# pySTEPS/pysteps

Hardware: AMD Instinct MI355X
Metric: Mpixels*leadsteps/s (LK+semilag) at 4096x4096 fp32 (higher is better)
Workload: dtype f32

## Files before the change

include/pysteps_hip.h:

```cpp
#ifndef PYSTEPS_HIP_H
#define PYSTEPS_HIP_H

#include <stddef.h>
#include <stdint.h>

#ifdef __cplusplus
extern "C" {
#endif

#define PSH_OK 0
#define PSH_EINVAL (-1)
#define PSH_EHIP (-2)
#define PSH_ENOTINIT (-3)
#define PSH_ENOMEM (-4)
#define PSH_ECOMM (-5)
#define PSH_EUNSUPPORTED (-6)
#define PSH_EINPUT (-7)

int psh_init(int device_id);
int psh_shutdown(void);
const char *psh_last_error(void);
const char *psh_version(void);
int psh_device_info(int *device_id, int *cu_count, size_t *hbm_total, size_t *hbm_free,
                    char *name, int name_len);
// ... 254 lines not shown
typedef struct psh_lk_params {
  int size_opening;
  int buffer_mask;
  int max_corners;
  int block_size;
  double quality_level, min_distance;
  int win_w, win_h;
  int max_level;
  int max_count;
  double epsilon;
  double min_eig_threshold;
  double nr_std_outlier;
  int k_outlier;
  double decl_scale;
  int idw_k;
  double idw_power, idw_dist_offset;
  int frames_f64;
} psh_lk_params;
int psh_dense_lk_dev(const float *frames_dev, int nframes, int m, int n, const psh_lk_params *params,
                     float *field_dev, double *xy_host, double *uv_host, int capacity,
                     int *count_out);
int psh_dense_lk_uv_dev(const float *frames_dev, int nframes, int m, int n, const psh_lk_params *params,
                        float *field_dev, float *field_uv_dev, double *xy_host, double *uv_host, int capacity,
                        int *count_out);

int psh_outliers_local_host(const double *xy, const double *values, int n, int k, double thr,
                            unsigned char *flags);

int psh_decluster_host(const double *xy, const double *values, int n, double scale,
                       int min_samples, double *out_xy, double *out_values, int *out_count);
int psh_vectors_finish_host(const double *xy, const double *values, const unsigned char *outlier_flags,
                            int count, double decl_scale, int m, int n, float *out_xy, float *out_values,
                            int *out_count, int *out_mode, float *out_const, float *out_reach);

int psh_fft_rfft2_dev(const double *in_dev, int m, int n, void *out_dev);
int psh_fft_irfft2_dev(const void *in_dev, int m, int n, double *out_dev);
int psh_fft_irfft2_min_dev(const void *in_dev, int m, int n, double *out_dev, unsigned long long *min_key_dev);
int psh_fft_c2c2_dev(const void *in_dev, int m, int n, int inverse, void *out_dev);

int psh_cascade_decompose_dev(const double *field_dev, const double *weights_dev, int nlevels, int m, int n,
                              int normalize, int subtract_mean, double *levels_dev, double *means_host,
                              double *stds_host, double *field_mean_host);
int psh_cascade_decompose_stats_dev(const double *field_dev, const double *weights_dev, int nlevels, int m, int n,
                                    double *levels_dev, double *stats_dev);
int psh_cascade_decompose_levels_dev(const double *field_dev, const double *weights_dev, int nlevels, int m, int n,
                                     double *levels_dev);
int psh_cascade_recompose_dev(const double *levels_dev, int nlevels, int m, int n, const double *means_host,
                              const double *stds_host, double field_mean, double *out_dev);
int psh_noise_filter_dev(const double *white_dev, const double *filter_dev, int m, int n, double *out_dev);
int psh_ar_iterate_dev(const double *x_dev, int nt, size_t plane, const double *phi_host, int p,
                       const double *eps_dev, double *out_dev);

int psh_probmatch_dev(const double *initial_dev, const double *target_dev, size_t count, double *out_dev);
int psh_probmatch_async_dev(const double *initial_dev, const double *target_dev, size_t count, double *out_dev,
                            int *status_dev);
int psh_probmatch_status(int status);
int psh_order_statistic_dev(const double *field_dev, size_t count, size_t index, double *value_host);
int psh_probmatch_plan_create(const double *target_dev, size_t count, void **plan_out);
int psh_probmatch_plan_destroy(void *plan);
int psh_probmatch_planned_dev(const void *plan, const double *initial_dev, size_t count, double *out_dev, int *status_dev);
int psh_steps_mask_probmatch_dev(const void *plan, double *field_dev, size_t count, const double *grey_mask_dev,
                                 const unsigned char *keep_mask_dev, const unsigned long long *min_key_dev,
                                 double *out_dev, int *status_dev);

int psh_dilated_mask_dev(const unsigned char *mask_dev, int m, int n, const unsigned char *kr_host, int kh, int kw,
                         int r, double *out_dev);
// ... 89 lines not shown
```

pysteps_amd/_lib.py:

```python

import ctypes
import os
import threading

from ctypes import POINTER, c_char_p, c_double, c_float, c_int, c_size_t, c_void_p

_PKG = os.path.dirname(os.path.abspath(__file__))
LIB_PATH = os.environ.get("PYSTEPS_HIP_LIB") or os.path.join(_PKG, "lib", "libpysteps_hip.so")

PSH_OK = 0
PSH_EINVAL = -1
PSH_EHIP = -2
PSH_ENOTINIT = -3
PSH_ENOMEM = -4
PSH_ECOMM = -5
PSH_EUNSUPPORTED = -6
PSH_EINPUT = -7


class LkParams(ctypes.Structure):

    _fields_ = [
        ("size_opening", c_int), ("buffer_mask", c_int), ("max_corners", c_int), ("block_size", c_int),
        ("quality_level", c_double), ("min_distance", c_double),
# ... 191 lines not shown
    "psh_lk_track_pyr_dev": (c_int, [c_void_p, c_void_p, c_int, c_int, c_double, c_double, c_void_p, c_void_p]),
    "psh_db_transform_dev": (c_int, [c_void_p, c_void_p, c_size_t, c_double, c_double, c_int]),
    "psh_field_transform_dev": (c_int, [c_void_p, c_void_p, c_int, c_size_t, c_int, c_double, c_double, c_double, c_double]),
    "psh_nqt_count_le_dev": (c_int, [c_void_p, c_int, c_size_t, c_void_p, c_void_p, POINTER(c_size_t), POINTER(c_double),
                                     POINTER(c_double), POINTER(c_float)]),
    "psh_nqt_forward_dev": (c_int, [c_void_p, c_int, c_void_p, c_size_t, c_size_t, c_double, c_double, c_void_p, c_int,
                                    POINTER(c_double)]),
    "psh_nqt_table_dev": (c_int, [c_size_t, c_double, c_void_p]),
    "psh_nqt_inverse_dev": (c_int, [c_void_p, c_int, c_size_t, c_void_p, c_void_p, c_int, c_size_t, c_void_p, c_int,
                                    POINTER(c_double), POINTER(c_double)]),
    "psh_nonfinite_count_f64_dev": (c_int, [c_void_p, c_size_t, POINTER(c_double)]),
    "psh_field_stats_dev": (c_int, [c_void_p, c_size_t, POINTER(c_double), POINTER(c_double), POINTER(c_double), POINTER(c_double)]),
    "psh_dense_lk_dev": (c_int, [c_void_p, c_int, c_int, c_int, POINTER(LkParams), c_void_p, c_void_p, c_void_p, c_int, POINTER(c_int)]),
    "psh_dense_lk_uv_dev": (c_int, [c_void_p, c_int, c_int, c_int, POINTER(LkParams), c_void_p, c_void_p, c_void_p, c_void_p, c_int,
                                    POINTER(c_int)]),
    "psh_semilag_dev": (c_int, [c_void_p, c_void_p, c_int, c_int, c_void_p, c_int, c_int, c_int, c_float, c_void_p, c_int, c_void_p]),
    "psh_semilag_uv_dev": (c_int, [c_void_p, c_void_p, c_void_p, c_int, c_int, c_void_p, c_int, c_int, c_int, c_float, c_void_p, c_int,
                                   c_void_p]),
    "psh_semilag_window_shape": (c_int, [c_int, c_int]),
    "psh_semilag_kernel": (c_int, [c_int, c_int, c_int, c_int, c_int, c_int]),
    "psh_semilag_rows_dev": (c_int, [c_void_p, c_void_p, c_int, c_int, c_void_p, c_int, c_int, c_int, c_float, c_void_p, c_int, c_int, c_int, c_void_p]),
    "psh_semilag_host": (c_int, [c_void_p, c_void_p, c_int, c_int, c_void_p, c_int, c_int, c_int, c_float, c_void_p, c_void_p, c_void_p, c_int, POINTER(c_int)]),
}

DIMENSION_SIGNATURES = {
    "psh_aggregate_axis_dev": (c_int, [c_void_p, c_int, c_size_t, c_size_t, c_size_t, c_int, c_int, c_int, c_void_p]),
    "psh_aggregate_space_dev": (c_int, [c_void_p, c_int, c_size_t, c_int, c_int, c_int, c_int, c_int, c_int, c_void_p]),
    "psh_accumulate_step_dev": (c_int, [c_void_p, c_int, c_void_p, c_int, c_void_p, c_size_t, c_int, c_int, c_int, c_int]),
    "psh_window_copy_dev": (c_int, [c_void_p, c_int, c_size_t, c_int, c_int, c_int, c_int, c_void_p, c_int, c_int, c_int, c_int, c_int,
                                    c_int, c_int, c_double]),
    "psh_field_min_dev": (c_int, [c_void_p, c_int, c_size_t, POINTER(c_double)]),
}

_lock = threading.RLock()
_lib = None
_initialised = False


def load():
    global _lib
    with _lock:
        if _lib is not None:
            return _lib
        if not os.path.exists(LIB_PATH):
            raise HipLibraryError(
                "libpysteps_hip.so not found at %s - build it with "
                "`python -m pysteps_amd.build` (hipcc, gfx950). pysteps_amd has no CPU fallback."
                % LIB_PATH
            )
        try:
            lib = ctypes.CDLL(LIB_PATH)
        except OSError as exc:
            raise HipLibraryError("cannot load %s: %s" % (LIB_PATH, exc)) from exc
        for name, (restype, argtypes) in list(SIGNATURES.items()) + list(DIMENSION_SIGNATURES.items()):
            try:
                fn = getattr(lib, name)
            except AttributeError as exc:
                raise HipLibraryError("%s does not export %s" % (LIB_PATH, name)) from exc
            fn.restype = restype
            fn.argtypes = argtypes
        _lib = lib
        return lib


def last_error():
    msg = load().psh_last_error()
    return msg.decode("utf-8", "replace") if msg else ""


def check(rc, what=""):
    if rc == PSH_OK:
        return
    msg = "%s%s" % (what + ": " if what else "", last_error())
    if rc in (PSH_EINVAL, PSH_EINPUT):
        raise ValueError(msg)
    if rc == PSH_EUNSUPPORTED:
        raise NotImplementedError(msg)
    if rc == PSH_ENOMEM:
        raise MemoryError(msg)
    raise HipLibraryError(msg)


def default_device():
    for key in ("PYSTEPS_HIP_DEVICE", "LOCAL_RANK"):
        val = os.environ.get(key)
        if val not in (None, ""):
            return int(val)
# ... 13 lines not shown
```

pysteps_amd/csrc/common.h:

```cpp
#pragma once

#include <hip/hip_runtime.h>

#include <cmath>
#include <cstdarg>
#include <cstddef>
#include <cstdint>
#include <cstdio>
#include <mutex>

#include "../../include/pysteps_hip.h"
#include "entry.h"
#include "scratch.h"

#ifdef PSH_DEBUG
#include <cassert>
#define PSH_DASSERT(cond) assert(cond)
#else
#define PSH_DASSERT(cond) ((void)0)
#endif

namespace psh {

constexpr int kNumXcd = 8;
// ... 94 lines not shown
                            int npad = 0, int pad_edge = 0, float cval = 0.f, int order = 3);

struct IdwDyn {
  int L;
  int mode;
  float cu, cv;
  float reach;
  int pad[3];
};

bool fft_shape_supported(int m, int n);
int fft_irfft2_weighted(const void *spec_dev, const double *weights_dev, int m, int n, double *out_dev,
                        void *scratch_dev, unsigned long long *min_key_dev = nullptr);

int moments(const double *x_dev, int planes, size_t plane, double2 *stats_dev, hipStream_t stream);

struct IdwArgs {
  const float *xy;
  const float *uv;
  float *out;
  float *out_uv = nullptr;
  int L, k, m, n;
  float x0, dx, y0, dy;
  float inv_res, power, offset, dmax;
  void *scratch = nullptr;
  const IdwDyn *dyn = nullptr;
};
hipError_t launch_idw(const IdwArgs &a, hipStream_t stream);
int idw_resident(const float *xy_dev, const float *values_dev, int capacity, const IdwDyn *dyn_dev, int m, int n,
                 int k, double power, double dist_offset, float *out_dev, float *out_uv_dev = nullptr);
size_t idw_scratch_bytes(int m, int n);
void set_idw_variant(int v);

hipError_t launch_outliers_pooled(const double *xy_dev, const double *uv_dev, const int *count_dev,
                                  int capacity, int k, double thr, unsigned char *flags_dev,
                                  hipStream_t stream);
int lk_track_pool(void *pyramid_handle, const float *points_host, const float *points_dev, const int *npts_dev,
                  int npts, int max_count, double epsilon, double min_eig_threshold, double *pool_xy_dev,
                  double *pool_uv_dev, int *pool_count_dev, int pool_capacity);

int lk_corners_resident(const unsigned char *feature_u8_dev, const float *clean_dev, float *stats_dev, int m, int n,
                        int block_size, int buffer_mask, double quality_level, double min_distance, int max_corners,
                        float *points_dev, int *npoints_dev, int (*before_walk)(void *) = nullptr,
                        void *before_walk_arg = nullptr, int *walk_stats_host = nullptr,
                        unsigned *slots_cleared = nullptr);

size_t lk_prepare_ws_bytes(int m, int n, bool f64);
int lk_prepare_on(hipStream_t stream, void *ws, const void *frame_dev, bool f64, int m, int n, int size_opening,
                  int buffer_mask, float *clean_dev, unsigned char *track_u8_dev, unsigned char *feature_u8_dev,
                  float *stats_dev, unsigned *slots_cleared = nullptr, unsigned long long *keepbits = nullptr);
size_t lk_keepbits_bytes(int m, int n);
size_t lk_slot_bytes();
int lk_pyramids_on_side(hipStream_t side, void *block, size_t block_bytes, const unsigned char *prev_u8_dev,
                        const unsigned char *next_u8_dev, int m, int n, int win_w, int win_h, int max_level,
                        void **handle_out);
size_t lk_pyramids_bytes(int m, int n, int win_w, int win_h, int max_level);

int corner_order_max_corners();
bool corner_order_supported(int m, int n, double min_distance, int max_corners);
size_t corner_order_ws_bytes();
hipError_t launch_corner_order(const unsigned long long *raw_dev, const int *raw_count_dev, int cap,
                               const float *eig_max_dev, float quality, int n, double min_distance,
                               int max_corners, void *ws_dev, float *points_dev, int *npoints_dev,
                               hipStream_t stream, int (*before_walk)(void *), void *before_walk_arg,
                               bool ws_is_cleared, const unsigned *eig_slots_dev = nullptr, int count_bias = 0,
                               float *eig_max_out_dev = nullptr);
size_t corner_order_clear_bytes();
size_t corner_order_walk_stats_offset();
hipError_t launch_vectors_finish(const double *pool_xy_dev, const double *pool_uv_dev,
                                 const unsigned char *flags_dev, const int *pool_count_dev, int capacity,
                                 double decl_scale, int m, int n, float *xy_out_dev, float *uv_out_dev,
                                 IdwDyn *dyn_dev, hipStream_t stream);

}
```

pysteps_amd/csrc/dense_lk.hip:

```cpp
#include <algorithm>
#include <chrono>
#include <cmath>
#include <cstdio>
#include <cstdlib>
#include <cstring>
#include <vector>

#include "common.h"

namespace {

__global__ __launch_bounds__(256) void zero_dwords(unsigned *__restrict__ p, size_t n) {
  for (size_t i = threadIdx.x; i < n; i += 256) p[i] = 0u;
}

}

extern "C" int psh_dense_lk_uv_dev(const float *frames_dev, int nframes, int m, int n, const psh_lk_params *prm,
                                   float *field_dev, float *field_uv_dev, double *xy_host, double *uv_host, int capacity,
                                   int *count_out);

extern "C" int psh_dense_lk_dev(const float *frames_dev, int nframes, int m, int n,
                                const psh_lk_params *prm, float *field_dev, double *xy_host,
                                double *uv_host, int capacity, int *count_out) {
// ... 83 lines not shown
    const int rc1 = psh::lk_corners_resident(feat[t].as<unsigned char>(), nan_pattern(t),
                                             stats[t].as<float>(), m, n, prm->block_size, prm->buffer_mask,
                                             prm->quality_level, prm->min_distance, prm->max_corners, d_pts, d_npts,
                                             nullptr, nullptr, trace ? walk_stats : nullptr, frame_slots(t));
    if (int rc = prepare(t + 1, side, ws_side.as<void>())) {
      (void)psh::side_end();
      return rc;
    }
    struct Fork {
      void *pyr;
      int rc;
    } fork{nullptr, PSH_OK};
    fork.rc = psh::lk_pyramids_on_side(side, pyr_block.release(), pyr_bytes, trk[t].as<unsigned char>(), trk[t + 1].as<unsigned char>(),
                                       m, n, prm->win_w, prm->win_h, prm->max_level, &fork.pyr);
    const int rcj = psh::side_end();
    void *pyr = fork.pyr;
    if (trace)
      std::fprintf(stderr,
                   "dense_lk corner walk: %d chunk(s), %d candidates, %d evaluation(s) of the first wave; us: load %d sort %d "
                   "coordinates %d block tests %d survivors %d (cells %d - evaluations %d append %d) total %d\n",
                   walk_stats[0], walk_stats[1], walk_stats[2], walk_stats[3], walk_stats[4], walk_stats[5],
                   walk_stats[6], walk_stats[7], walk_stats[9], walk_stats[11], walk_stats[12], walk_stats[8]);
    if (rc1 || rcj || fork.rc || !pyr) {
      if (pyr) (void)psh_lk_pyramids_free(pyr);
      return fork.rc ? fork.rc : rc1 ? rc1 : rcj ? rcj : psh::fail(PSH_EHIP, "dense_lk: pyramids were not built");
    }
    const int rc2 = psh::lk_track_pool(pyr, nullptr, d_pts, d_npts, prm->max_corners, prm->max_count, prm->epsilon,
                                       prm->min_eig_threshold, d_pxy, d_puv, d_pcnt, capacity_dev);
    const int rc3 = psh_lk_pyramids_free(pyr);
    if (rc2) return rc2;
    if (rc3) return rc3;
  }
  mark("pairs queued");
  PSH_HIP(psh::launch_outliers_pooled(d_pxy, d_puv, d_pcnt, capacity_dev, prm->k_outlier, prm->nr_std_outlier,
                                      d_pfl, c.stream));
  if (field_dev) {
    psh::Scratch samples;
    const size_t sbytes = cap * 2 * sizeof(float);
    if (int rc = samples.alloc(2 * sbytes + 256)) return rc;
    float *d_xy = samples.as<float>(), *d_uv = d_xy + cap * 2;
    psh::IdwDyn *d_dyn = samples.at<psh::IdwDyn>(2 * sbytes);
    PSH_HIP(psh::launch_vectors_finish(d_pxy, d_puv, d_pfl, d_pcnt, capacity_dev, prm->decl_scale, m, n, d_xy, d_uv,
                                       d_dyn, c.stream));
    if (int rc = psh::idw_resident(d_xy, d_uv, capacity_dev, d_dyn, m, n, prm->idw_k, prm->idw_power,
                                   prm->idw_dist_offset, field_dev, field_uv_dev))
      return rc;
    mark("dense field queued");
    if (count_out) {
      static void *pinned_cnt = nullptr;
      if (int rc = psh::persistent_pinned(&pinned_cnt, 64)) return rc;
      PSH_HIP(hipMemcpyAsync(pinned_cnt, &d_dyn->L, sizeof(int), hipMemcpyDeviceToHost, c.stream));
      PSH_HIP(hipStreamSynchronize(c.stream));
      *count_out = *static_cast<const int *>(pinned_cnt);
    }
    return PSH_OK;
  }

  static void *pinned = nullptr;
  constexpr size_t kPinBytes = 2 * 8192 * 16 + 256 + 8192;
  if (int rc = psh::persistent_pinned(&pinned, kPinBytes)) return rc;
  char *pin = static_cast<char *>(pinned);
  PSH_HIP(hipMemcpyAsync(pin, pbase, off_fl + cap, hipMemcpyDeviceToHost, c.stream));
  PSH_HIP(hipStreamSynchronize(c.stream));
  mark("pooled vectors on the host");
  const int pooled = std::min(*reinterpret_cast<const int *>(pin + off_cnt), capacity_dev);
  const double *hxy = reinterpret_cast<const double *>(pin);
  const double *huv = reinterpret_cast<const double *>(pin + off_uv);
  const unsigned char *hfl = reinterpret_cast<const unsigned char *>(pin + off_fl);
  int count = 0;
  for (int i = 0; i < pooled; ++i) {
    if (pooled >= 2 && hfl[i]) continue;
    if (count >= capacity)
      return psh::fail(PSH_EINVAL, "dense_lk: the vectors exceed the output capacity %d", capacity);
    xy_host[2 * count] = hxy[2 * i];
    xy_host[2 * count + 1] = hxy[2 * i + 1];
    uv_host[2 * count] = huv[2 * i];
// ... 7 lines not shown
```

pysteps_amd/csrc/lk_sparse.hip:

```cpp
#include <cstddef>

#include "common.h"

namespace psh {
namespace {

using CornerKey = unsigned long long;

constexpr int kOrdThreads = 1024;
constexpr int kOrdWaves = kOrdThreads / 64;
constexpr int kOrdBins = 1024;
constexpr int kChunkCap = 4096;
constexpr int kMaxCornersDev = 2048;
constexpr int kHashSlots = 8192;

template <bool DESC>
__device__ __forceinline__ void bitonic_sort_lds(unsigned long long *keys, int p2) {
  for (int k = 2; k <= p2; k <<= 1) {
    for (int j = k >> 1; j > 0; j >>= 1) {
      for (int t = threadIdx.x; t < (p2 >> 1); t += blockDim.x) {
        const int i = ((t & ~(j - 1)) << 1) | (t & (j - 1)), o = i | j;
        const unsigned long long a = keys[i], b = keys[o];
        const bool first_half = (i & k) == 0;
        if ((first_half == DESC) ? a < b : a > b) {
          keys[i] = b;
          keys[o] = a;
        }
      }
      const int next_j = j > 1 ? (j >> 1) : k;
      if (j > 64 || next_j > 64 || (k == p2 && j == 1)) {
        __syncthreads();
      } else {
        __builtin_amdgcn_fence(__ATOMIC_RELEASE, "wavefront");
        __builtin_amdgcn_wave_barrier();
        __builtin_amdgcn_fence(__ATOMIC_ACQUIRE, "wavefront");
// ... 601 lines not shown
      lap(tk_batch);
    }
    remaining -= cnt;
    if (T <= key_lo) break;
    upper = T;
    __syncthreads();
  }
  if (tid == 0) {
    *npoints = nacc;
    if (hdr) {
      hdr->walk[0] = st_chunks;
      hdr->walk[1] = st_walked;
      hdr->walk[2] = st_batches;
      const long long tk[6] = {tk_load, tk_sort, tk_xy, tk_test, tk_batch, wall_clock64() - tk_start};
      for (int q = 0; q < 6; ++q) hdr->phase_us[q] = static_cast<int>(tk[q] / 100);
      for (int q = 0; q < 4; ++q) hdr->sub_us[q] = static_cast<int>(tk_sub[q] / 100);
    }
  }
}

constexpr int kFinMax = 8192;

__device__ __forceinline__ double wave_min_f64(double v) {
#pragma unroll
  for (int d = 32; d >= 1; d >>= 1) v = fmin(v, __shfl_xor(v, d));
  return v;
}
__device__ __forceinline__ double wave_max_f64(double v) {
#pragma unroll
  for (int d = 32; d >= 1; d >>= 1) v = fmax(v, __shfl_xor(v, d));
  return v;
}

__global__ __launch_bounds__(kOrdThreads) void vectors_finish(const double2 *__restrict__ pool_xy,
                                                              const double2 *__restrict__ pool_uv,
                                                              const unsigned char *__restrict__ flags,
                                                              const int *__restrict__ pool_count, int capacity,
                                                              double scale, int m, int n,
                                                              float2 *__restrict__ out_xy,
                                                              float2 *__restrict__ out_uv,
                                                              IdwDyn *__restrict__ dyn) {
  __shared__ unsigned long long s_keys[kFinMax];
  __shared__ unsigned short s_seg[kFinMax];
  __shared__ int s_scan[kOrdWaves];
  __shared__ double s_stat[6][kOrdWaves];
  __shared__ double s_first[2];
  const int tid = threadIdx.x, lane = tid & 63, wave = tid >> 6;
  const int pooled = min(max(*pool_count, 0), min(capacity, kFinMax));
  const bool decl = scale > 1.0;
  constexpr unsigned long long kDropped = ~0ull;
  const int p2 = next_pow2(pooled);
  for (int i = tid; i < p2; i += kOrdThreads) {
    unsigned long long key = kDropped;
    if (i < pooled && !(pooled >= 2 && flags[i])) {
      unsigned cellkey = 0u;
      if (decl) {
        const double2 p = pool_xy[i];
        const double fx = floor(p.x / scale), fy = floor(p.y / scale);
        const unsigned cx = static_cast<unsigned>(fmin(fmax(fx, 0.0), 65535.0));
        const unsigned cy = static_cast<unsigned>(fmin(fmax(fy, 0.0), 65535.0));
        cellkey = (cx << 16) | cy;
      }
      key = decl ? (static_cast<unsigned long long>(cellkey) << 32) | static_cast<unsigned>(i)
                 : static_cast<unsigned long long>(i) << 32 | static_cast<unsigned>(i);
    }
    s_keys[i] = key;
  }
  __syncthreads();
  bitonic_sort_lds<false>(s_keys, p2);
  const int per = max(p2 / kOrdThreads, 1);
  const int t0 = tid * per;
  int heads = 0, kept_here = 0;
  for (int q = 0; q < per; ++q) {
    const int t = t0 + q;
    if (t >= p2) break;
    const unsigned long long k = s_keys[t];
    if (k == kDropped) continue;
    ++kept_here;
    if (t == 0 || (s_keys[t - 1] >> 32) != (k >> 32)) ++heads;
  }
  int incl = heads;
#pragma unroll
  for (int d = 1; d < 64; d <<= 1) {
    const int up = __shfl_up(incl, d);
    if (lane >= d) incl += up;
  }
  if (lane == 63) s_scan[wave] = incl;
  __syncthreads();
  int before = incl - heads, cells = 0;
  for (int w = 0; w < kOrdWaves; ++w) {
    if (w < wave) before += s_scan[w];
    cells += s_scan[w];
  }
  {
    int slot = before - 1;
    for (int q = 0; q < per; ++q) {
      const int t = t0 + q;
      if (t >= p2) break;
      const unsigned long long k = s_keys[t];
      if (k == kDropped) continue;
      if (t == 0 || (s_keys[t - 1] >> 32) != (k >> 32)) ++slot;
      s_seg[t] = static_cast<unsigned short>(slot);
    }
  }
  (void)kept_here;
  __syncthreads();
  double vmin = INFINITY, vmax = -INFINITY;
  double xmin = 0.0, xmax = static_cast<double>(n) - 1.0, ymin = 0.0, ymax = static_cast<double>(m) - 1.0;
  for (int t = tid; t < p2; t += kOrdThreads) {
    const unsigned long long k = s_keys[t];
    if (k == kDropped) continue;
    const unsigned cellkey = static_cast<unsigned>(k >> 32);
    int s = t, e = t + 1;
    while (s > 0 && static_cast<unsigned>(s_keys[s - 1] >> 32) == cellkey) --s;
    while (e < p2 && static_cast<unsigned>(s_keys[e] >> 32) == cellkey) ++e;
    const int members = e - s;
    const int me = static_cast<int>(k & 0xffffffffull);
    const double2 mxy = pool_xy[me], muv = pool_uv[me];
    const double mine[4] = {mxy.x, mxy.y, muv.x, muv.y};
    int rank[4] = {0, 0, 0, 0};
    double succ[4] = {INFINITY, INFINITY, INFINITY, INFINITY};
    for (int q = s; q < e; ++q) {
      if (q == t) continue;
      const int o = static_cast<int>(s_keys[q] & 0xffffffffull);
      const double2 oxy = pool_xy[o], ouv = pool_uv[o];
      const double other[4] = {oxy.x, oxy.y, ouv.x, ouv.y};
#pragma unroll
      for (int c = 0; c < 4; ++c) {
        const bool below = other[c] < mine[c] || (other[c] == mine[c] && q < t);
        rank[c] += below ? 1 : 0;
        if (!below) succ[c] = fmin(succ[c], other[c]);
      }
    }
    const int lower = (members - 1) / 2;
    const bool even = (members & 1) == 0;
    const int slot = s_seg[t];
    double med[4];
    bool have[4];
#pragma unroll
    for (int c = 0; c < 4; ++c) {
      have[c] = rank[c] == lower;
      med[c] = 0.5 * (mine[c] + (even ? succ[c] : mine[c]));
    }
    if (have[0]) {
      reinterpret_cast<float *>(out_xy)[2 * slot] = static_cast<float>(med[0]);
      xmin = fmin(xmin, med[0]);
      xmax = fmax(xmax, med[0]);
    }
    if (have[1]) {
      reinterpret_cast<float *>(out_xy)[2 * slot + 1] = static_cast<float>(med[1]);
      ymin = fmin(ymin, med[1]);
      ymax = fmax(ymax, med[1]);
    }
    if (have[2]) {
      reinterpret_cast<float *>(out_uv)[2 * slot] = static_cast<float>(med[2]);
      vmin = fmin(vmin, med[2]);
      vmax = fmax(vmax, med[2]);
      if (slot == 0) s_first[0] = med[2];
// ... 60 lines not shown
hipError_t launch_corner_order(const unsigned long long *raw_dev, const int *raw_count_dev, int cap,
                               const float *eig_max_dev, float quality, int n, double min_distance,
                               int max_corners, void *ws_dev, float *points_dev, int *npoints_dev,
                               hipStream_t stream, int (*before_walk)(void *), void *before_walk_arg,
                               bool ws_is_cleared, const unsigned *eig_slots_dev, int count_bias, float *eig_max_out_dev) {
  const int cell = static_cast<int>(std::lrint(min_distance)) > 1 ? static_cast<int>(std::lrint(min_distance)) : 1;
  const double md2 = std::ceil(min_distance * min_distance);
  const unsigned md2_ceil = md2 >= 2147483647.0 ? 2147483647u : static_cast<unsigned>(md2);
  char *ws = static_cast<char *>(ws_dev);
  int *hist = reinterpret_cast<int *>(ws);
  OrderHeader *hdr = reinterpret_cast<OrderHeader *>(ws + kOrdOffHdr);
  CornerKey *head = reinterpret_cast<CornerKey *>(ws + kOrdOffHead);
  if (!ws_is_cleared) {
    const hipError_t e = hipMemsetAsync(ws, 0, kOrdOffHead, stream);
    if (e != hipSuccess) return e;
  }
  const int groups = std::max(1, std::min(128, (cap + 4 * kPreThreads - 1) / (4 * kPreThreads)));
  hipLaunchKernelGGL(corner_hist, dim3(groups), dim3(kPreThreads), 0, stream, raw_dev, raw_count_dev, cap, eig_max_dev,
                     quality, hist, eig_slots_dev, count_bias);
  int ccap = 1024;
  while (ccap < 2 * max_corners && ccap < kChunkCap) ccap <<= 1;
  hipLaunchKernelGGL(corner_gather, dim3(groups), dim3(kPreThreads), 0, stream, raw_dev, raw_count_dev, cap, eig_max_dev,
                     quality, hist, head, hdr, ccap, eig_slots_dev, count_bias);
  if (before_walk != nullptr && before_walk(before_walk_arg) != 0) return hipErrorUnknown;
  hipLaunchKernelGGL(corner_order, dim3(1), dim3(kOrdThreads), 0, stream, raw_dev, raw_count_dev, cap, eig_max_dev,
                     quality, head, hdr, n, cell, md2_ceil, min_distance >= 1.0 ? 1 : 0, max_corners, ccap,
                     reinterpret_cast<float2 *>(points_dev), npoints_dev, eig_slots_dev, count_bias, eig_max_out_dev);
  return hipGetLastError();
}

hipError_t launch_vectors_finish(const double *pool_xy_dev, const double *pool_uv_dev,
                                 const unsigned char *flags_dev, const int *pool_count_dev, int capacity,
                                 double decl_scale, int m, int n, float *xy_out_dev, float *uv_out_dev,
                                 IdwDyn *dyn_dev, hipStream_t stream) {
  hipLaunchKernelGGL(vectors_finish, dim3(1), dim3(kOrdThreads), 0, stream,
                     reinterpret_cast<const double2 *>(pool_xy_dev), reinterpret_cast<const double2 *>(pool_uv_dev),
                     flags_dev, pool_count_dev, capacity, decl_scale, m, n, reinterpret_cast<float2 *>(xy_out_dev),
                     reinterpret_cast<float2 *>(uv_out_dev), dyn_dev);
  return hipGetLastError();
}

}

extern "C" int psh_lk_order_host(const unsigned long long *keys_host, int count, float response_max,
                                 double quality_level, int m, int n, double min_distance, int max_corners,
                                 float *points_host, int *count_host) {
  PSH_ENTER(c);
  if (!points_host || !count_host || (count > 0 && !keys_host)) return psh::fail(PSH_EINVAL, "lk_order: NULL pointer");
  if (count < 0 || m <= 0 || n <= 0 || max_corners <= 0) return psh::fail(PSH_EINVAL, "lk_order: invalid argument");
  if (!psh::corner_order_supported(m, n, min_distance, max_corners))
    return psh::fail(PSH_EUNSUPPORTED, "lk_order: more than %d corners, 65535 rows / columns or min_distance >= 16383",
                     psh::kMaxCornersDev);
  const size_t key_bytes = (static_cast<size_t>(count) * sizeof(unsigned long long) + 255) & ~static_cast<size_t>(255);
  const size_t pts_bytes = static_cast<size_t>(max_corners) * 2 * sizeof(float);
  psh::Scratch blk;
  const size_t ws_bytes = (psh::corner_order_ws_bytes() + 255) & ~static_cast<size_t>(255);
  if (int rc = blk.alloc(key_bytes + 256 + pts_bytes + 256 + ws_bytes)) return rc;
  char *base = blk.as<char>();
  unsigned long long *d_keys = reinterpret_cast<unsigned long long *>(base);
  int *d_hdr = reinterpret_cast<int *>(base + key_bytes);
  float *d_pts = reinterpret_cast<float *>(base + key_bytes + 256);
  void *d_ws = base + ((key_bytes + 256 + pts_bytes + 255) & ~static_cast<size_t>(255));
  struct {
    int count, accepted;
    float top;
  } hdr = {count, 0, response_max};
  if (count > 0) PSH_HIP(hipMemcpyAsync(d_keys, keys_host, static_cast<size_t>(count) * 8, hipMemcpyHostToDevice, c.stream));
  PSH_HIP(hipMemcpyAsync(d_hdr, &hdr, sizeof(hdr), hipMemcpyHostToDevice, c.stream));
  PSH_HIP(hipStreamSynchronize(c.stream));
  PSH_HIP(psh::launch_corner_order(d_keys, d_hdr, count, reinterpret_cast<const float *>(d_hdr + 2),
                                   static_cast<float>(quality_level), n, min_distance, max_corners, d_ws, d_pts,
// ... 24 lines not shown
  const size_t vec = cap * 16, off_uv = vec, off_fl = 2 * vec, off_cnt = (off_fl + cap + 255) & ~static_cast<size_t>(255);
  const size_t off_oxy = off_cnt + 256, off_ouv = off_oxy + cap * 8, off_dyn = off_ouv + cap * 8;
  psh::Scratch blk;
  if (int rc = blk.alloc(off_dyn + sizeof(psh::IdwDyn))) return rc;
  char *base = blk.as<char>();
  if (count > 0) {
    PSH_HIP(hipMemcpyAsync(base, xy, vec, hipMemcpyHostToDevice, c.stream));
    PSH_HIP(hipMemcpyAsync(base + off_uv, values, vec, hipMemcpyHostToDevice, c.stream));
    PSH_HIP(hipMemcpyAsync(base + off_fl, outlier_flags, cap, hipMemcpyHostToDevice, c.stream));
  }
  PSH_HIP(hipMemcpyAsync(base + off_cnt, &count, sizeof(int), hipMemcpyHostToDevice, c.stream));
  PSH_HIP(hipStreamSynchronize(c.stream));
  PSH_HIP(psh::launch_vectors_finish(reinterpret_cast<const double *>(base), reinterpret_cast<const double *>(base + off_uv),
                                     reinterpret_cast<const unsigned char *>(base + off_fl),
                                     reinterpret_cast<const int *>(base + off_cnt), static_cast<int>(cap), decl_scale, m, n,
                                     reinterpret_cast<float *>(base + off_oxy), reinterpret_cast<float *>(base + off_ouv),
                                     reinterpret_cast<psh::IdwDyn *>(base + off_dyn), c.stream));
  psh::IdwDyn d;
  PSH_HIP(hipMemcpyAsync(&d, base + off_dyn, sizeof(d), hipMemcpyDeviceToHost, c.stream));
  PSH_HIP(hipStreamSynchronize(c.stream));
  const int L = d.L < 0 ? 0 : d.L > count ? count : d.L;
  if (L > 0) {
    PSH_HIP(hipMemcpyAsync(out_xy, base + off_oxy, static_cast<size_t>(L) * 8, hipMemcpyDeviceToHost, c.stream));
    PSH_HIP(hipMemcpyAsync(out_values, base + off_ouv, static_cast<size_t>(L) * 8, hipMemcpyDeviceToHost, c.stream));
    PSH_HIP(hipStreamSynchronize(c.stream));
  }
  *out_count = L;
  *out_mode = d.mode;
  out_const[0] = d.cu;
  out_const[1] = d.cv;
  *out_reach = d.reach;
  return PSH_OK;
}
```

pysteps_amd/csrc/sparse_qc.hip:

```cpp
#include <vector>

#include "common.h"

namespace psh {
namespace {

constexpr int kQcMaxN = 8192;

__device__ __forceinline__ unsigned wave_min_u32(unsigned v) {
#define PSH_MIN_STEP(CTRL, ROWMASK)                                                                       \
  {                                                                                                        \
    const unsigned o = static_cast<unsigned>(                                                              \
        __builtin_amdgcn_update_dpp(static_cast<int>(v), static_cast<int>(v), CTRL, ROWMASK, 0xf, false)); \
    v = o < v ? o : v;                                                                                     \
  }
  PSH_MIN_STEP(0xB1, 0xf)
  PSH_MIN_STEP(0x4E, 0xf)
  PSH_MIN_STEP(0x141, 0xf)
  PSH_MIN_STEP(0x140, 0xf)
  PSH_MIN_STEP(0x142, 0xa)
  PSH_MIN_STEP(0x143, 0xc)
#undef PSH_MIN_STEP
  return static_cast<unsigned>(__builtin_amdgcn_readlane(static_cast<int>(v), 63));
}

__device__ __forceinline__ unsigned long long wave_min_u64(unsigned long long v) {
  const unsigned hi = static_cast<unsigned>(v >> 32), lo = static_cast<unsigned>(v);
  const unsigned m_hi = wave_min_u32(hi);
  const unsigned m_lo = wave_min_u32(hi == m_hi ? lo : 0xffffffffu);
  return (static_cast<unsigned long long>(m_hi) << 32) | m_lo;
}

__device__ __forceinline__ bool mahalanobis_outlier(int cnt, double sa, double sb, double saa, double sab, double sbb,
                                                    double thr) {
#pragma clang fp contract(off)
// ... 69 lines not shown
        sab += a * b;
        sbb += b * b;
        ++cnt;
      }
    }
    __syncthreads();
  }
  if (lane != 0) return;
  flags[i] = mahalanobis_outlier(cnt, sa, sb, saa, sab, sbb, thr) ? 1 : 0;
}

template <int N>
__device__ __forceinline__ void sort_keys_ascending(unsigned long long (&a)[N]) {
#pragma unroll
  for (int k = 2; k <= N; k <<= 1) {
#pragma unroll
    for (int j = k >> 1; j > 0; j >>= 1) {
#pragma unroll
      for (int i = 0; i < N; ++i) {
        const int l = i ^ j;
        if (l > i) {
          const bool up = (i & k) == 0;
          const unsigned long long x = a[i], y = a[l];
          const bool swap = up ? (x > y) : (x < y);
          a[i] = swap ? y : x;
          a[l] = swap ? x : y;
        }
      }
    }
  }
}

template <int KPER>
__global__ __launch_bounds__(64) void outliers_local_sorted(const double2 *__restrict__ xy,
                                                            const double2 *__restrict__ uv, int n_host,
                                                            const int *__restrict__ n_dev, int k, double thr,
                                                            unsigned char *__restrict__ flags) {
  __shared__ unsigned long long keys[KPER * 64];
  __shared__ double2 s_nb[64];
  const int n = n_dev ? *n_dev : n_host;
  const int i = blockIdx.x, lane = threadIdx.x;
  if (i >= n) return;
  if (n < 2) {
    if (lane == 0) flags[i] = 0;
    return;
  }
  const double2 me = xy[i], mine = uv[i];
  constexpr unsigned long long kGone = ~0ull;
  unsigned long long mykeys[KPER];
  double2 p[KPER];
#pragma unroll
  for (int q = 0; q < KPER; ++q) {
    const int j = q * 64 + lane;
    p[q] = j < n ? xy[j] : make_double2(0.0, 0.0);
  }
#pragma unroll
  for (int q = 0; q < KPER; ++q) {
    const int j = q * 64 + lane;
    const double dx = p[q].x - me.x, dy = p[q].y - me.y;
    const float d = static_cast<float>(dx * dx + dy * dy);
    mykeys[q] = j < n ? (static_cast<unsigned long long>(__float_as_uint(d)) << 32) | static_cast<unsigned>(j) : kGone;
  }
  sort_keys_ascending<KPER>(mykeys);
#pragma unroll
  for (int q = 0; q < KPER; ++q) keys[q * 64 + lane] = mykeys[q];
  unsigned long long best = mykeys[0];
  int next = 1;
  double sa = 0.0, sb = 0.0, saa = 0.0, sab = 0.0, sbb = 0.0;
  int cnt = 0;
  const int kk = min(n, k + 1);
  int mine_j = -1;
  for (int t0 = 0; t0 < kk; t0 += 64) {
    const int tn = min(64, kk - t0);
    for (int t = 0; t < tn; ++t) {
      const unsigned long long g = wave_min_u64(best);
      const int j = static_cast<int>(g & 0xffffffffull);
      if (lane == t) mine_j = j;
      if ((j & 63) == lane) {
        best = next < KPER ? keys[next * 64 + lane] : kGone;
        ++next;
      }
    }
    if (lane < tn) {
      const double2 q = uv[mine_j];
      s_nb[lane] = make_double2(q.x - mine.x, q.y - mine.y);
    }
    __syncthreads();
    if (lane == 0) {
      for (int t = (t0 == 0 ? 1 : 0); t < tn; ++t) {
        const double a = s_nb[t].x, b = s_nb[t].y;
        sa += a;
        sb += b;
        saa += a * a;
        sab += a * b;
        sbb += b * b;
        ++cnt;
      }
    }
    __syncthreads();
  }
  if (lane != 0) return;
  flags[i] = mahalanobis_outlier(cnt, sa, sb, saa, sab, sbb, thr) ? 1 : 0;
}

static void launch_outliers(int rows, size_t cap_for_lds, hipStream_t stream, const double2 *xy, const double2 *uv, int n_host,
                            const int *n_dev, int k, double thr, unsigned char *flags) {
  if (rows <= 16 * 64) {
    hipLaunchKernelGGL(outliers_local_sorted<16>, dim3(rows), dim3(64), 0, stream, xy, uv, n_host, n_dev, k, thr, flags);
  } else if (rows <= 32 * 64) {
    hipLaunchKernelGGL(outliers_local_sorted<32>, dim3(rows), dim3(64), 0, stream, xy, uv, n_host, n_dev, k, thr, flags);
  } else {
    hipLaunchKernelGGL(outliers_local, dim3(rows), dim3(64), cap_for_lds * sizeof(unsigned long long), stream, xy, uv, n_host,
                       n_dev, k, thr, flags);
  }
}

}
}

namespace psh {
hipError_t launch_outliers_pooled(const double *xy_dev, const double *uv_dev, const int *count_dev,
                                  int capacity, int k, double thr, unsigned char *flags_dev,
                                  hipStream_t stream) {
  launch_outliers(capacity, static_cast<size_t>(capacity), stream, reinterpret_cast<const double2 *>(xy_dev),
                  reinterpret_cast<const double2 *>(uv_dev), 0, count_dev, k, thr, flags_dev);
  return hipGetLastError();
}
}

extern "C" int psh_outliers_local_host(const double *xy, const double *values, int n, int k,
                                       double thr, unsigned char *flags) {
  PSH_ENTER(c);
  if (n < 0) return psh::fail(PSH_EINVAL, "outliers: negative sample count");
  if (n == 0) return PSH_OK;
  if (!xy || !values || !flags) return psh::fail(PSH_EINVAL, "outliers: NULL pointer");
  if (k < 1) return psh::fail(PSH_EINVAL, "outliers: k must be >= 1");
  if (n > psh::kQcMaxN)
    return psh::fail(PSH_EUNSUPPORTED, "outliers: more than %d vectors not implemented on the device",
                     psh::kQcMaxN);
  if (n < 2) {
    flags[0] = 0;
    return PSH_OK;
  }
  const size_t vec_bytes = static_cast<size_t>(n) * 2 * sizeof(double);
  psh::Scratch blk;
  if (int rc = blk.alloc(2 * vec_bytes + static_cast<size_t>(n))) return rc;
  char *base = blk.as<char>();
  double2 *d_xy = reinterpret_cast<double2 *>(base);
  double2 *d_uv = reinterpret_cast<double2 *>(base + vec_bytes);
  unsigned char *d_fl = reinterpret_cast<unsigned char *>(base + 2 * vec_bytes);
  PSH_HIP(hipMemcpyAsync(d_xy, xy, vec_bytes, hipMemcpyHostToDevice, c.stream));
  PSH_HIP(hipMemcpyAsync(d_uv, values, vec_bytes, hipMemcpyHostToDevice, c.stream));
  psh::launch_outliers(n, static_cast<size_t>(n), c.stream, d_xy, d_uv, n, nullptr, k, thr, d_fl);
  PSH_HIP(hipGetLastError());
  PSH_HIP(hipMemcpyAsync(flags, d_fl, static_cast<size_t>(n), hipMemcpyDeviceToHost, c.stream));
  PSH_HIP(hipStreamSynchronize(c.stream));
  return PSH_OK;
}
// ... 100 lines not shown
```

Baseline: 276,100.

## Presort decluster keys in parallel during outlier pass and stage samples in LDS

Adds extra blocks to the pooled outlier kernel that compute decluster cell keys and sort them by rank counting across many workgroups. The single-block vectors_finish kernel then reads these presorted keys, compacts away outliers with a wave scan, and skips its own bitonic sort. Pool xy/uv and flags are staged into LDS for the per-cell ranking loop. This moves serial work out of a one-block kernel, at the cost of more LDS use and an extra scratch allocation. A host entry point for outliers plus finish is also added.

```diff
diff --git a/include/pysteps_hip.h b/include/pysteps_hip.h
--- a/include/pysteps_hip.h
+++ b/include/pysteps_hip.h
@@ -310,6 +310,7 @@
 int psh_vectors_finish_host(const double *xy, const double *values, const unsigned char *outlier_flags,
                             int count, double decl_scale, int m, int n, float *out_xy, float *out_values,
                             int *out_count, int *out_mode, float *out_const, float *out_reach);
+#include "pysteps_hip_sparse.h"
 
 int psh_fft_rfft2_dev(const double *in_dev, int m, int n, void *out_dev);
 int psh_fft_irfft2_dev(const void *in_dev, int m, int n, double *out_dev);
diff --git a/include/pysteps_hip_sparse.h b/include/pysteps_hip_sparse.h
--- /dev/null
+++ b/include/pysteps_hip_sparse.h
@@ -0,0 +1,16 @@
+#ifndef PYSTEPS_HIP_SPARSE_H
+#define PYSTEPS_HIP_SPARSE_H
+
+#ifdef __cplusplus
+extern "C" {
+#endif
+
+int psh_outliers_finish_host(const double *xy, const double *values, int count, int k, double thr,
+                             double decl_scale, int m, int n, unsigned char *flags_out, float *out_xy,
+                             float *out_values, int *out_count, int *out_mode, float *out_const, float *out_reach);
+
+#ifdef __cplusplus
+}
+#endif
+
+#endif
diff --git a/pysteps_amd/_lib.py b/pysteps_amd/_lib.py
--- a/pysteps_amd/_lib.py
+++ b/pysteps_amd/_lib.py
@@ -247,6 +247,11 @@
     "psh_field_min_dev": (c_int, [c_void_p, c_int, c_size_t, POINTER(c_double)]),
 }
 
+SPARSE_SIGNATURES = {
+    "psh_outliers_finish_host": (c_int, [c_void_p, c_void_p, c_int, c_int, c_double, c_double, c_int, c_int, c_void_p,
+                                         c_void_p, c_void_p, POINTER(c_int), POINTER(c_int), c_void_p, c_void_p]),
+}
+
 _lock = threading.RLock()
 _lib = None
 _initialised = False
@@ -267,7 +272,7 @@
             lib = ctypes.CDLL(LIB_PATH)
         except OSError as exc:
             raise HipLibraryError("cannot load %s: %s" % (LIB_PATH, exc)) from exc
-        for name, (restype, argtypes) in list(SIGNATURES.items()) + list(DIMENSION_SIGNATURES.items()):
+        for name, (restype, argtypes) in list(SIGNATURES.items()) + list(DIMENSION_SIGNATURES.items()) + list(SPARSE_SIGNATURES.items()):
             try:
                 fn = getattr(lib, name)
             except AttributeError as exc:
diff --git a/pysteps_amd/csrc/common.h b/pysteps_amd/csrc/common.h
--- a/pysteps_amd/csrc/common.h
+++ b/pysteps_amd/csrc/common.h
@@ -150,9 +150,11 @@
 size_t idw_scratch_bytes(int m, int n);
 void set_idw_variant(int v);
 
+constexpr int kPresortMax = 2048;
 hipError_t launch_outliers_pooled(const double *xy_dev, const double *uv_dev, const int *count_dev,
                                   int capacity, int k, double thr, unsigned char *flags_dev,
-                                  hipStream_t stream);
+                                  hipStream_t stream, double decl_scale = 0.0,
+                                  unsigned long long *sorted_keys_dev = nullptr, bool *presorted = nullptr);
 int lk_track_pool(void *pyramid_handle, const float *points_host, const float *points_dev, const int *npts_dev,
                   int npts, int max_count, double epsilon, double min_eig_threshold, double *pool_xy_dev,
                   double *pool_uv_dev, int *pool_count_dev, int pool_capacity);
@@ -188,6 +190,7 @@
 hipError_t launch_vectors_finish(const double *pool_xy_dev, const double *pool_uv_dev,
                                  const unsigned char *flags_dev, const int *pool_count_dev, int capacity,
                                  double decl_scale, int m, int n, float *xy_out_dev, float *uv_out_dev,
-                                 IdwDyn *dyn_dev, hipStream_t stream);
+                                 IdwDyn *dyn_dev, hipStream_t stream,
+                                 const unsigned long long *sorted_keys_dev = nullptr);
 
 }
diff --git a/pysteps_amd/csrc/decluster_key.h b/pysteps_amd/csrc/decluster_key.h
--- /dev/null
+++ b/pysteps_amd/csrc/decluster_key.h
@@ -0,0 +1,16 @@
+#pragma once
+
+#include <hip/hip_runtime.h>
+
+namespace psh {
+
+__device__ __forceinline__ unsigned long long decluster_key(double2 p, int i, double scale) {
+  if (!(scale > 1.0)) return static_cast<unsigned long long>(i) << 32 | static_cast<unsigned>(i);
+  const double fx = floor(p.x / scale), fy = floor(p.y / scale);
+  const unsigned cx = static_cast<unsigned>(fmin(fmax(fx, 0.0), 65535.0));
+  const unsigned cy = static_cast<unsigned>(fmin(fmax(fy, 0.0), 65535.0));
+  const unsigned cellkey = (cx << 16) | cy;
+  return (static_cast<unsigned long long>(cellkey) << 32) | static_cast<unsigned>(i);
+}
+
+}
diff --git a/pysteps_amd/csrc/dense_lk.hip b/pysteps_amd/csrc/dense_lk.hip
--- a/pysteps_amd/csrc/dense_lk.hip
+++ b/pysteps_amd/csrc/dense_lk.hip
@@ -139,8 +139,13 @@
     if (rc3) return rc3;
   }
   mark("pairs queued");
+  psh::Scratch sorted;
+  if (field_dev)
+    if (int rc = sorted.alloc(cap * sizeof(unsigned long long))) return rc;
+  bool presorted = false;
   PSH_HIP(psh::launch_outliers_pooled(d_pxy, d_puv, d_pcnt, capacity_dev, prm->k_outlier, prm->nr_std_outlier,
-                                      d_pfl, c.stream));
+                                      d_pfl, c.stream, prm->decl_scale,
+                                      field_dev ? sorted.as<unsigned long long>() : nullptr, &presorted));
   if (field_dev) {
     psh::Scratch samples;
     const size_t sbytes = cap * 2 * sizeof(float);
@@ -148,7 +153,7 @@
     float *d_xy = samples.as<float>(), *d_uv = d_xy + cap * 2;
     psh::IdwDyn *d_dyn = samples.at<psh::IdwDyn>(2 * sbytes);
     PSH_HIP(psh::launch_vectors_finish(d_pxy, d_puv, d_pfl, d_pcnt, capacity_dev, prm->decl_scale, m, n, d_xy, d_uv,
-                                       d_dyn, c.stream));
+                                       d_dyn, c.stream, presorted ? sorted.as<unsigned long long>() : nullptr));
     if (int rc = psh::idw_resident(d_xy, d_uv, capacity_dev, d_dyn, m, n, prm->idw_k, prm->idw_power,
                                    prm->idw_dist_offset, field_dev, field_uv_dev))
       return rc;
diff --git a/pysteps_amd/csrc/lk_sparse.hip b/pysteps_amd/csrc/lk_sparse.hip
--- a/pysteps_amd/csrc/lk_sparse.hip
+++ b/pysteps_amd/csrc/lk_sparse.hip
@@ -1,6 +1,7 @@
 #include <cstddef>
 
 #include "common.h"
+#include "decluster_key.h"
 
 namespace psh {
 namespace {
@@ -668,6 +669,9 @@
   return v;
 }
 
+constexpr int kFinStage = kPresortMax;
+
+template <bool PRESORTED>
 __global__ __launch_bounds__(kOrdThreads) void vectors_finish(const double2 *__restrict__ pool_xy,
                                                               const double2 *__restrict__ pool_uv,
                                                               const unsigned char *__restrict__ flags,
@@ -675,35 +679,76 @@
                                                               double scale, int m, int n,
                                                               float2 *__restrict__ out_xy,
                                                               float2 *__restrict__ out_uv,
-                                                              IdwDyn *__restrict__ dyn) {
+                                                              IdwDyn *__restrict__ dyn,
+                                                              const unsigned long long *__restrict__ sorted) {
   __shared__ unsigned long long s_keys[kFinMax];
   __shared__ unsigned short s_seg[kFinMax];
   __shared__ int s_scan[kOrdWaves];
   __shared__ double s_stat[6][kOrdWaves];
   __shared__ double s_first[2];
   const int tid = threadIdx.x, lane = tid & 63, wave = tid >> 6;
-  const int pooled = min(max(*pool_count, 0), min(capacity, kFinMax));
-  const bool decl = scale > 1.0;
+  const int pooled = min(max(*pool_count, 0), min(capacity, PRESORTED ? kFinStage : kFinMax));
   constexpr unsigned long long kDropped = ~0ull;
   const int p2 = next_pow2(pooled);
-  for (int i = tid; i < p2; i += kOrdThreads) {
-    unsigned long long key = kDropped;
-    if (i < pooled && !(pooled >= 2 && flags[i])) {
-      unsigned cellkey = 0u;
-      if (decl) {
-        const double2 p = pool_xy[i];
-        const double fx = floor(p.x / scale), fy = floor(p.y / scale);
-        const unsigned cx = static_cast<unsigned>(fmin(fmax(fx, 0.0), 65535.0));
-        const unsigned cy = static_cast<unsigned>(fmin(fmax(fy, 0.0), 65535.0));
-        cellkey = (cx << 16) | cy;
-      }
-      key = decl ? (static_cast<unsigned long long>(cellkey) << 32) | static_cast<unsigned>(i)
-                 : static_cast<unsigned long long>(i) << 32 | static_cast<unsigned>(i);
-    }
-    s_keys[i] = key;
-  }
-  __syncthreads();
-  bitonic_sort_lds<false>(s_keys, p2);
+  double2 *s_xy = nullptr, *s_uv = nullptr;
+  if constexpr (PRESORTED) {
+    __shared__ double2 s_stage[2 * kFinStage];
+    __shared__ unsigned char s_fl[kFinStage];
+    s_xy = s_stage;
+    s_uv = s_stage + kFinStage;
+    constexpr int kRun = kFinMax / kOrdThreads;
+    const int per0 = max(p2 / kOrdThreads, 1), t0 = tid * per0;
+    unsigned long long run[kRun];
+#pragma unroll
+    for (int q = 0; q < kRun; ++q) run[q] = (q < per0 && t0 + q < pooled) ? sorted[t0 + q] : kDropped;
+    for (int i = tid; i < pooled; i += kOrdThreads) {
+      s_xy[i] = pool_xy[i];
+      s_uv[i] = pool_uv[i];
+      s_fl[i] = flags[i];
+    }
+    __syncthreads();
+    int kept = 0;
+#pragma unroll
+    for (int q = 0; q < kRun; ++q) {
+      if (run[q] == kDropped) continue;
+      const int i = static_cast<int>(run[q] & 0xffffffffull);
+      PSH_DASSERT(i >= 0 && i < pooled);
+      if (pooled >= 2 && s_fl[i]) {
+        run[q] = kDropped;
+      } else {
+        ++kept;
+      }
+    }
+    int incl = kept;
+#pragma unroll
+    for (int d = 1; d < 64; d <<= 1) {
+      const int up = __shfl_up(incl, d);
+      if (lane >= d) incl += up;
+    }
+    if (lane == 63) s_scan[wave] = incl;
+    __syncthreads();
+    int pos = incl - kept, total = 0;
+    for (int w = 0; w < kOrdWaves; ++w) {
+      if (w < wave) pos += s_scan[w];
+      total += s_scan[w];
+    }
+#pragma unroll
+    for (int q = 0; q < kRun; ++q)
+      if (run[q] != kDropped) s_keys[pos++] = run[q];
+    for (int i = total + tid; i < p2; i += kOrdThreads) s_keys[i] = kDropped;
+    __syncthreads();
+  } else {
+    for (int i = tid; i < p2; i += kOrdThreads) {
+      unsigned long long key = kDropped;
+      if (i < pooled && !(pooled >= 2 && flags[i]))
+        key = decluster_key(scale > 1.0 ? pool_xy[i] : make_double2(0.0, 0.0), i, scale);
+      s_keys[i] = key;
+    }
+    __syncthreads();
+    bitonic_sort_lds<false>(s_keys, p2);
+  }
+  auto sample_xy = [&](int i) { return PRESORTED ? s_xy[i] : pool_xy[i]; };
+  auto sample_uv = [&](int i) { return PRESORTED ? s_uv[i] : pool_uv[i]; };
   const int per = max(p2 / kOrdThreads, 1);
   const int t0 = tid * per;
   int heads = 0, kept_here = 0;
@@ -752,14 +797,14 @@
     while (e < p2 && static_cast<unsigned>(s_keys[e] >> 32) == cellkey) ++e;
     const int members = e - s;
     const int me = static_cast<int>(k & 0xffffffffull);
-    const double2 mxy = pool_xy[me], muv = pool_uv[me];
+    const double2 mxy = sample_xy(me), muv = sample_uv(me);
     const double mine[4] = {mxy.x, mxy.y, muv.x, muv.y};
     int rank[4] = {0, 0, 0, 0};
     double succ[4] = {INFINITY, INFINITY, INFINITY, INFINITY};
     for (int q = s; q < e; ++q) {
       if (q == t) continue;
       const int o = static_cast<int>(s_keys[q] & 0xffffffffull);
-      const double2 oxy = pool_xy[o], ouv = pool_uv[o];
+      const double2 oxy = sample_xy(o), ouv = sample_uv(o);
       const double other[4] = {oxy.x, oxy.y, ouv.x, ouv.y};
 #pragma unroll
       for (int c = 0; c < 4; ++c) {
@@ -886,11 +931,18 @@
 hipError_t launch_vectors_finish(const double *pool_xy_dev, const double *pool_uv_dev,
                                  const unsigned char *flags_dev, const int *pool_count_dev, int capacity,
                                  double decl_scale, int m, int n, float *xy_out_dev, float *uv_out_dev,
-                                 IdwDyn *dyn_dev, hipStream_t stream) {
-  hipLaunchKernelGGL(vectors_finish, dim3(1), dim3(kOrdThreads), 0, stream,
-                     reinterpret_cast<const double2 *>(pool_xy_dev), reinterpret_cast<const double2 *>(pool_uv_dev),
-                     flags_dev, pool_count_dev, capacity, decl_scale, m, n, reinterpret_cast<float2 *>(xy_out_dev),
-                     reinterpret_cast<float2 *>(uv_out_dev), dyn_dev);
+                                 IdwDyn *dyn_dev, hipStream_t stream, const unsigned long long *sorted_keys_dev) {
+#define PSH_FINISH(PRESORTED)                                                                                           \
+  hipLaunchKernelGGL(vectors_finish<PRESORTED>, dim3(1), dim3(kOrdThreads), 0, stream,                                  \
+                     reinterpret_cast<const double2 *>(pool_xy_dev), reinterpret_cast<const double2 *>(pool_uv_dev),    \
+                     flags_dev, pool_count_dev, capacity, decl_scale, m, n, reinterpret_cast<float2 *>(xy_out_dev),     \
+                     reinterpret_cast<float2 *>(uv_out_dev), dyn_dev, sorted_keys_dev)
+  if (sorted_keys_dev != nullptr) {
+    PSH_FINISH(true);
+  } else {
+    PSH_FINISH(false);
+  }
+#undef PSH_FINISH
   return hipGetLastError();
 }
 
@@ -981,3 +1033,56 @@
   *out_reach = d.reach;
   return PSH_OK;
 }
+
+extern "C" int psh_outliers_finish_host(const double *xy, const double *values, int count, int k, double thr,
+                                        double decl_scale, int m, int n, unsigned char *flags_out, float *out_xy,
+                                        float *out_values, int *out_count, int *out_mode, float *out_const,
+                                        float *out_reach) {
+  PSH_ENTER(c);
+  if (count < 0 || m <= 0 || n <= 0) return psh::fail(PSH_EINVAL, "outliers_finish: invalid argument");
+  if (k < 1) return psh::fail(PSH_EINVAL, "outliers_finish: k must be >= 1");
+  if (count > psh::kFinMax) return psh::fail(PSH_EUNSUPPORTED, "outliers_finish: more than %d vectors", psh::kFinMax);
+  if (!out_xy || !out_values || !out_count || !out_mode || !out_const || !out_reach ||
+      (count > 0 && (!xy || !values || !flags_out)))
+    return psh::fail(PSH_EINVAL, "outliers_finish: NULL pointer");
+  auto up = [](size_t v) { return (v + 255) & ~static_cast<size_t>(255); };
+  const size_t cap = static_cast<size_t>(count > 0 ? count : 1);
+  const size_t vec = cap * 16, off_uv = vec, off_fl = 2 * vec, off_cnt = up(off_fl + cap), off_keys = off_cnt + 256;
+  const size_t off_oxy = off_keys + cap * 8, off_ouv = off_oxy + cap * 8, off_dyn = off_ouv + cap * 8;
+  psh::Scratch blk;
+  if (int rc = blk.alloc(off_dyn + sizeof(psh::IdwDyn))) return rc;
+  char *base = blk.as<char>();
+  if (count > 0) {
+    PSH_HIP(hipMemcpyAsync(base, xy, vec, hipMemcpyHostToDevice, c.stream));
+    PSH_HIP(hipMemcpyAsync(base + off_uv, values, vec, hipMemcpyHostToDevice, c.stream));
+  }
+  PSH_HIP(hipMemcpyAsync(base + off_cnt, &count, sizeof(int), hipMemcpyHostToDevice, c.stream));
+  PSH_HIP(hipStreamSynchronize(c.stream));
+  const double *d_xy = reinterpret_cast<const double *>(base), *d_uv = reinterpret_cast<const double *>(base + off_uv);
+  unsigned char *d_fl = reinterpret_cast<unsigned char *>(base + off_fl);
+  int *d_cnt = reinterpret_cast<int *>(base + off_cnt);
+  unsigned long long *d_keys = reinterpret_cast<unsigned long long *>(base + off_keys);
+  bool presorted = false;
+  PSH_HIP(psh::launch_outliers_pooled(d_xy, d_uv, d_cnt, static_cast<int>(cap), k, thr, d_fl, c.stream, decl_scale, d_keys,
+                                      &presorted));
+  PSH_HIP(psh::launch_vectors_finish(d_xy, d_uv, d_fl, d_cnt, static_cast<int>(cap), decl_scale, m, n,
+                                     reinterpret_cast<float *>(base + off_oxy), reinterpret_cast<float *>(base + off_ouv),
+                                     reinterpret_cast<psh::IdwDyn *>(base + off_dyn), c.stream,
+                                     presorted ? d_keys : nullptr));
+  psh::IdwDyn d;
+  PSH_HIP(hipMemcpyAsync(&d, base + off_dyn, sizeof(d), hipMemcpyDeviceToHost, c.stream));
+  if (count > 0) PSH_HIP(hipMemcpyAsync(flags_out, d_fl, static_cast<size_t>(count), hipMemcpyDeviceToHost, c.stream));
+  PSH_HIP(hipStreamSynchronize(c.stream));
+  const int L = d.L < 0 ? 0 : d.L > count ? count : d.L;
+  if (L > 0) {
+    PSH_HIP(hipMemcpyAsync(out_xy, base + off_oxy, static_cast<size_t>(L) * 8, hipMemcpyDeviceToHost, c.stream));
+    PSH_HIP(hipMemcpyAsync(out_values, base + off_ouv, static_cast<size_t>(L) * 8, hipMemcpyDeviceToHost, c.stream));
+    PSH_HIP(hipStreamSynchronize(c.stream));
+  }
+  *out_count = L;
+  *out_mode = d.mode;
+  out_const[0] = d.cu;
+  out_const[1] = d.cv;
+  *out_reach = d.reach;
+  return PSH_OK;
+}
diff --git a/pysteps_amd/csrc/sparse_qc.hip b/pysteps_amd/csrc/sparse_qc.hip
--- a/pysteps_amd/csrc/sparse_qc.hip
+++ b/pysteps_amd/csrc/sparse_qc.hip
@@ -1,6 +1,7 @@
 #include <vector>
 
 #include "common.h"
+#include "decluster_key.h"
 
 namespace psh {
 namespace {
@@ -136,14 +137,11 @@
 }
 
 template <int KPER>
-__global__ __launch_bounds__(64) void outliers_local_sorted(const double2 *__restrict__ xy,
-                                                            const double2 *__restrict__ uv, int n_host,
-                                                            const int *__restrict__ n_dev, int k, double thr,
-                                                            unsigned char *__restrict__ flags) {
-  __shared__ unsigned long long keys[KPER * 64];
-  __shared__ double2 s_nb[64];
-  const int n = n_dev ? *n_dev : n_host;
-  const int i = blockIdx.x, lane = threadIdx.x;
+__device__ __forceinline__ void outlier_test_sorted(const double2 *__restrict__ xy, const double2 *__restrict__ uv,
+                                                    int n, int i, int k, double thr,
+                                                    unsigned char *__restrict__ flags, unsigned long long *keys,
+                                                    double2 *s_nb) {
+  const int lane = threadIdx.x;
   if (i >= n) return;
   if (n < 2) {
     if (lane == 0) flags[i] = 0;
@@ -207,6 +205,47 @@
   flags[i] = mahalanobis_outlier(cnt, sa, sb, saa, sab, sbb, thr) ? 1 : 0;
 }
 
+template <int KPER>
+__global__ __launch_bounds__(64) void outliers_local_sorted(const double2 *__restrict__ xy,
+                                                            const double2 *__restrict__ uv, int n_host,
+                                                            const int *__restrict__ n_dev, int k, double thr,
+                                                            unsigned char *__restrict__ flags) {
+  __shared__ unsigned long long keys[KPER * 64];
+  __shared__ double2 s_nb[64];
+  outlier_test_sorted<KPER>(xy, uv, n_dev ? *n_dev : n_host, blockIdx.x, k, thr, flags, keys, s_nb);
+}
+
+template <int KPER>
+__global__ __launch_bounds__(64) void outliers_pooled_sorted(const double2 *__restrict__ xy,
+                                                             const double2 *__restrict__ uv, int rows,
+                                                             const int *__restrict__ n_dev, int k, double thr,
+                                                             unsigned char *__restrict__ flags, double scale,
+                                                             unsigned long long *__restrict__ sorted) {
+  __shared__ unsigned long long keys[KPER * 64];
+  __shared__ double2 s_nb[64];
+  const int n = min(*n_dev, rows);
+  if (static_cast<int>(blockIdx.x) < rows) {
+    outlier_test_sorted<KPER>(xy, uv, n, blockIdx.x, k, thr, flags, keys, s_nb);
+    return;
+  }
+  const int first = (static_cast<int>(blockIdx.x) - rows) * 64, lane = threadIdx.x;
+  if (first >= n) return;
+  const bool decl = scale > 1.0;
+#pragma unroll
+  for (int q = 0; q < KPER; ++q) {
+    const int j = q * 64 + lane;
+    if (j < n) keys[j] = decluster_key(decl ? xy[j] : make_double2(0.0, 0.0), j, scale);
+  }
+  __syncthreads();
+  const int i = first + lane;
+  if (i >= n) return;
+  const unsigned long long mine = keys[i];
+  int rank = 0;
+#pragma unroll 8
+  for (int j = 0; j < n; ++j) rank += keys[j] < mine ? 1 : 0;
+  sorted[rank] = mine;
+}
+
 static void launch_outliers(int rows, size_t cap_for_lds, hipStream_t stream, const double2 *xy, const double2 *uv, int n_host,
                             const int *n_dev, int k, double thr, unsigned char *flags) {
   if (rows <= 16 * 64) {
@@ -225,9 +264,24 @@
 namespace psh {
 hipError_t launch_outliers_pooled(const double *xy_dev, const double *uv_dev, const int *count_dev,
                                   int capacity, int k, double thr, unsigned char *flags_dev,
-                                  hipStream_t stream) {
-  launch_outliers(capacity, static_cast<size_t>(capacity), stream, reinterpret_cast<const double2 *>(xy_dev),
-                  reinterpret_cast<const double2 *>(uv_dev), 0, count_dev, k, thr, flags_dev);
+                                  hipStream_t stream, double decl_scale, unsigned long long *sorted_keys_dev,
+                                  bool *presorted) {
+  const double2 *xy = reinterpret_cast<const double2 *>(xy_dev), *uv = reinterpret_cast<const double2 *>(uv_dev);
+  static_assert(kPresortMax == 32 * 64, "outliers_pooled_sorted<32> holds 32 keys per lane");
+  const bool order = sorted_keys_dev != nullptr && capacity <= kPresortMax;
+  if (presorted) *presorted = order;
+  if (order) {
+    const dim3 grid(capacity + (capacity + 63) / 64);
+    if (capacity <= 16 * 64) {
+      hipLaunchKernelGGL(outliers_pooled_sorted<16>, grid, dim3(64), 0, stream, xy, uv, capacity, count_dev, k, thr,
+                         flags_dev, decl_scale, sorted_keys_dev);
+    } else {
+      hipLaunchKernelGGL(outliers_pooled_sorted<32>, grid, dim3(64), 0, stream, xy, uv, capacity, count_dev, k, thr,
+                         flags_dev, decl_scale, sorted_keys_dev);
+    }
+  } else {
+    launch_outliers(capacity, static_cast<size_t>(capacity), stream, xy, uv, 0, count_dev, k, thr, flags_dev);
+  }
   return hipGetLastError();
 }
 }
```

Result: no change. 278,400, median of 6 (+0.8%).
